# antoniorizzoeng/climate-sim-mpi-cpp

Measured on AMD Instinct MI355X. Metric: Mcell-updates/sec (16384^2 fp64 advection-diffusion sweep), higher is better.
Workload: dtype f64

## Files before the change

### climate-sim-mpi-cpp_amd/__init__.py

```python
from __future__ import annotations

import collections
import ctypes as C
import os
import subprocess
import weakref

import numpy as np

HERE = os.path.dirname(os.path.abspath(__file__))
ROOT = os.path.dirname(HERE)
LIB_PATH = os.environ.get("CSIM_LIB") or os.path.join(HERE, "lib", "libcsim.so")
HEADER = os.path.join(ROOT, "include", "csim.h")

DIRICHLET, NEUMANN, PERIODIC = 0, 1, 2
LEFT, RIGHT, BOTTOM, TOP = 0, 1, 2, 3
NO_NEIGHBOR = -1
UNIQUE_ID_BYTES = 128
VARIANTS = {"auto": 0, "dpp": 1, "lds": 2, "naive": 3}

_BC_NAMES = {
    "dirichlet": DIRICHLET, "fixed": DIRICHLET,
    "neumann": NEUMANN, "noflux": NEUMANN, "zero-flux": NEUMANN,
    "periodic": PERIODIC, "period": PERIODIC,
# ... 55 lines not shown

def lib() -> C.CDLL:
    global _lib
    if _lib is not None:
        return _lib
    if not os.path.exists(LIB_PATH):
        raise FileNotFoundError(
            f"{LIB_PATH} is missing: run __graft_entry__.build() (there is no CPU fallback)")
    if os.environ.get("CSIM_PRELOAD_TORCH", "1") != "0":
        try:
            import torch
        except Exception:
            pass
    L = C.CDLL(LIB_PATH, mode=C.RTLD_GLOBAL)
    dp, ip, vp = C.POINTER(C.c_double), C.POINTER(C.c_int), C.c_void_p
    d, i = C.c_double, C.c_int
    sig = {
        "csim_last_error": (C.c_char_p, []),
        "csim_abi_version": (i, []),
        "csim_device_count": (i, [ip]),
        "csim_set_device": (i, [i]),
        "csim_device_name": (i, [C.c_char_p, C.c_size_t]),
        "csim_safe_dt": (d, [d] * 5),
        "csim_decomp_init": (i, [i, i, i, i, C.POINTER(Decomp)]),
        "csim_exchange_plan": (i, [C.POINTER(Decomp), i, C.POINTER(Msg), ip, C.POINTER(Msg), ip]),
        "csim_field_create": (i, [i, i, i, d, d, C.POINTER(vp)]),
        "csim_field_destroy": (i, [vp]),
        "csim_field_upload": (i, [vp, dp]),
        "csim_field_download": (i, [vp, dp]),
        "csim_field_download_interior": (i, [vp, dp]),
        "csim_field_fill": (i, [vp, d]),
        "csim_field_copy": (i, [vp, vp]),
        "csim_field_swap": (i, [vp, vp]),
        "csim_field_minmax": (i, [vp, dp]),
        "csim_field_sum": (i, [vp, dp]),
        "csim_field_linf_diff": (i, [vp, vp, dp]),
        "csim_apply_boundary": (i, [vp, ip, ip, d]),
        "csim_diffusion_step": (i, [vp, vp, d, d]),
        "csim_advection_step": (i, [vp, vp, d, d, d]),
        "csim_fused_step": (i, [vp, vp, d, d, d, d]),
        "csim_stepper_create": (i, [C.POINTER(Decomp), d, d, ip, d, C.POINTER(vp)]),
        "csim_stepper_destroy": (i, [vp]),
        "csim_comm_unique_id": (i, [vp, C.c_size_t]),
        "csim_stepper_comm_init": (i, [vp, vp, C.c_size_t]),
        "csim_stepper_upload": (i, [vp, dp]),
        "csim_stepper_download": (i, [vp, dp]),
# ... 65 lines not shown
        "csim_obs_network_observe": (i, [vp, i, C.c_ulonglong, C.c_uint, i]),
        "csim_obs_noise": (i, [C.c_ulonglong, C.c_uint, C.c_uint, dp]),
        "csim_ensemble_assimilate_network": (i, [vp, vp, d, i, i]),
        "csim_obs_network_fetch": (i, [vp, dp, dp, dp, dp, dp, dp]),
        "csim_obs_network_log": (i, [vp, i, C.POINTER(CsimObsCycle), ip]),
        "csim_obs_network_log_reset": (i, [vp]),
        "csim_obs_network_create_linear": (i, [vp, i, ip, ip, ip, ip, ip, dp, dp, d, i, i, C.POINTER(vp)]),
        "csim_obs_network_taps": (i, [vp, ip]),
        "csim_obs_linear_check": (i, [i, i, i, i, i, ip, ip, ip, ip, ip, dp]),
        "csim_obs_taps_bilinear": (i, [i, i, d, d, ip, ip, ip, ip, dp]),
        "csim_obs_taps_box": (i, [i, i, i, i, i, i, ip, ip, ip, dp]),
        "csim_obs_network_set_active": (i, [vp, C.POINTER(C.c_ubyte)]),
        "csim_ensemble_assimilate_screened": (i, [vp, vp, d, i, i, d]),
        "csim_obs_network_screen_log": (i, [vp, i, C.POINTER(CsimObsScreenCycle), ip]),
        "csim_obs_network_status": (i, [vp, C.POINTER(C.c_ubyte)]),
        "csim_obs_screen_decide": (i, [d, d, d, d, d, i, ip]),
        "csim_ensemble_set_option": (i, [vp, C.c_char_p, C.c_long]),
        "csim_ensemble_get_option": (i, [vp, C.c_char_p, C.POINTER(C.c_long)]),
        "csim_ensemble_plan": (i, [i, i, i, i, ip]),
        "csim_ensemble_sign_class": (i, [d, d, d, d, d, d, i, ip]),
        "csim_ensemble_classes": (i, [i, ip, ip]),
    }
    for name, (res, args) in sig.items():
        fn = getattr(L, name)
        fn.restype = res
        fn.argtypes = args
    _lib = L
    return L


def declared_symbols():
    import re
    txt = open(HEADER).read()
    return sorted(set(re.findall(r"\b(csim_[a-z0-9_]+)\s*\(", txt)))


def _ck(rc):
    if rc != 0:
        raise CsimError(rc, lib().csim_last_error().decode())


def _dp(a):
    assert a.dtype == np.float64 and a.flags["C_CONTIGUOUS"]
    return a.ctypes.data_as(C.POINTER(C.c_double))


# ... 11 lines not shown
def bc_codes(code: str):
    m = {"d": DIRICHLET, "n": NEUMANN, "p": PERIODIC}
    return [m[c] for c in code.lower()]


def device_count() -> int:
    n = C.c_int(0)
    _ck(lib().csim_device_count(C.byref(n)))
    return n.value


def set_device(dev: int) -> None:
    _ck(lib().csim_set_device(dev))


def device_name() -> str:
    buf = C.create_string_buffer(256)
    _ck(lib().csim_device_name(buf, 256))
    return buf.value.decode()


def safe_dt(dx, dy, vx, vy, D) -> float:
    return lib().csim_safe_dt(dx, dy, vx, vy, D)


def decomp_init(size, rank, nx_global, ny_global) -> Decomp:
    d = Decomp()
    _ck(lib().csim_decomp_init(size, rank, nx_global, ny_global, C.byref(d)))
    return d


def exchange_plan(dec: Decomp, depth: int):
    sends, recvs = (Msg * 8)(), (Msg * 8)()
    ns, nr = C.c_int(0), C.c_int(0)
    _ck(lib().csim_exchange_plan(C.byref(dec), depth, sends, C.byref(ns), recvs, C.byref(nr)))
    return ([(m.peer, m.dir, m.count) for m in sends[:ns.value]],
            [(m.peer, m.dir, m.count) for m in recvs[:nr.value]])


def pass_schedule(nsteps: int, smallest_tile: int = 1 << 30, fuse: int = -1, tile_cells: int = 0, diffusion_only: bool = False):
    n = C.c_long(0)
    args = (nsteps, min(smallest_tile, 1 << 30), tile_cells, fuse, int(diffusion_only))
    _ck(lib().csim_pass_schedule_for(*args, None, 0, C.byref(n)))
    buf = (C.c_int * max(1, n.value))()
    _ck(lib().csim_pass_schedule_for(*args, buf, n.value, C.byref(n)))
    return list(buf[:n.value])
# ... 776 lines not shown
```

### climate-sim-mpi-cpp_amd/csrc/api.cpp

```cpp
#include "stepper.hpp"

namespace csim {

static thread_local std::string g_err;
int fail(int code, const std::string& msg) {
    g_err = msg;
    return code;
}
static bool pow2(double x) {
    if (!(x > 0.0) || !std::isnormal(x)) return false;
    int e = 0;
    return std::frexp(x, &e) == 0.5 && std::isnormal(1.0 / x);
}

Phys make_phys(double dx, double dy, double D, double dt, double vx, double vy, bool contract) {
    Phys p;
    p.kdiff = dt * D;
    p.mdt = -dt;
    p.vx = vx;
    p.vy = vy;
    p.dx = dx;
    p.dy = dy;
    p.dx2 = dx * dx;
    p.dy2 = dy * dy;
// ... 4 lines not shown
    if (dx == 1.0 && dy == 1.0)
        p.div_mode = 0;
    else if (pow2(dx) && pow2(dy) && pow2(p.dx2) && pow2(p.dy2))
        p.div_mode = 1;
    else
        p.div_mode = 2;
    {
        const long double kx = static_cast<long double>(dt) * D / (static_cast<long double>(dx) * dx);
        const long double ky = static_cast<long double>(dt) * D / (static_cast<long double>(dy) * dy);
        const long double cx = static_cast<long double>(dt) * vx / dx, cy = static_cast<long double>(dt) * vy / dy;
        const long double acx = cx < 0 ? -cx : cx, acy = cy < 0 ? -cy : cy;
        p.a0 = static_cast<double>(1.0L - 2.0L * kx - 2.0L * ky - acx - acy);
        p.aW = static_cast<double>(kx + (vx >= 0.0 ? acx : 0.0L));
        p.aE = static_cast<double>(kx + (vx >= 0.0 ? 0.0L : acx));
        p.aS = static_cast<double>(ky + (vy >= 0.0 ? acy : 0.0L));
        p.aN = static_cast<double>(ky + (vy >= 0.0 ? 0.0L : acy));
    }
    {
        const double g = (1.0 + 4.0 * std::fabs(p.kdiff) * (1.0 / p.dx2 + 1.0 / p.dy2) +
                          2.0 * std::fabs(p.mdt) * (std::fabs(vx) / std::fabs(dx) + std::fabs(vy) / std::fabs(dy))) * (1.0 + 1e-9);
        const double thr = std::ldexp(1.0, 1022) / std::pow(g, MAX_FUSE);
        p.fast_thr = (std::isfinite(g) && thr >= std::ldexp(1.0, 900)) ? thr : 0.0;
    }
    if (contract) p.div_mode = 3;
    return p;
}

int finish_partials(const double* scratch_dev, int nblocks, int kind, double out[2],
                           hipStream_t st) {
    std::vector<double> h(2 * REDUCE_BLOCKS);
    CSIM_HIP(hipMemcpyAsync(h.data(), scratch_dev, sizeof(double) * 2 * REDUCE_BLOCKS,
                            hipMemcpyDeviceToHost, st));
    CSIM_HIP(hipStreamSynchronize(st));
    double r0 = h[0], r1 = h[REDUCE_BLOCKS];
    for (int k = 1; k < nblocks; ++k) {
        if (kind == 0) {
            r0 = std::fmin(r0, h[k]);
            r1 = std::fmax(r1, h[REDUCE_BLOCKS + k]);
        } else if (kind == 1) {
            r0 += h[k];
        } else {
            r0 = max_nan(r0, h[k]);
        }
    }
    out[0] = r0;
    out[1] = r1;
// ... 51 lines not shown

const char* csim_last_error(void) { return g_err.c_str(); }

int csim_abi_version(void) { return CSIM_ABI_VERSION; }

int csim_device_count(int* count) {
    CSIM_REQUIRE(count, "count is null");
    CSIM_HIP(hipGetDeviceCount(count));
    return CSIM_OK;
}

int csim_set_device(int device) {
    CSIM_HIP(hipSetDevice(device));
    return CSIM_OK;
}

int csim_device_name(char* buf, size_t n) {
    CSIM_REQUIRE(buf && n > 0, "bad buffer");
    int dev = 0;
    CSIM_HIP(hipGetDevice(&dev));
    hipDeviceProp_t prop;
    CSIM_HIP(hipGetDeviceProperties(&prop, dev));
    std::snprintf(buf, n, "%s", prop.gcnArchName);
    return CSIM_OK;
}

double csim_safe_dt(double dx, double dy, double vx, double vy, double D) {
    const double inf = std::numeric_limits<double>::infinity();
    const double ax = std::fabs(vx), ay = std::fabs(vy);
    const double rate = (ax > 0 ? ax / dx : 0.0) + (ay > 0 ? ay / dy : 0.0);
    const double dt_adv = rate > 0 ? 1.0 / rate : inf;
    const double w = 1.0 / (dx * dx) + 1.0 / (dy * dy);
    const double dt_diff = D > 0 ? 1.0 / (2.0 * D * w) : inf;
    return std::min(dt_adv, dt_diff);
}

int csim_decomp_init(int size, int rank, int nx_global, int ny_global, csim_decomp* out) {
    CSIM_REQUIRE(out, "out is null");
    CSIM_REQUIRE(size >= 1 && rank >= 0 && rank < size, "bad size/rank");
    CSIM_REQUIRE(nx_global > 0 && ny_global > 0, "nx/ny must be > 0");
    int small = 1;
    for (int f = 1; static_cast<long>(f) * f <= size; ++f)
        if (size % f == 0) small = f;
    csim_decomp d{};
    d.size = size;
    d.rank = rank;
// ... 190 lines not shown
```

### climate-sim-mpi-cpp_amd/csrc/internal.hpp

```cpp
#pragma once

#include <hip/hip_runtime.h>

#include <cstddef>
#include <cstdio>
#include <string>

#include "csim.h"

namespace csim {

constexpr int LPAD = 16;
constexpr int WAVE_COLS = 128;

inline int round_up(int v, int m) { return (v + m - 1) / m * m; }
inline int pitch_for(int nx) { return LPAD + round_up(nx + 1, WAVE_COLS) + WAVE_COLS; }

int fail(int code, const std::string& msg);

#define CSIM_HIP(expr)                                                                       \
    do {                                                                                     \
        hipError_t e_ = (expr);                                                              \
        if (e_ != hipSuccess)                                                                \
            return ::csim::fail(CSIM_ERR_HIP, std::string(#expr) + ": " + hipGetErrorString(e_)); \
    } while (0)

struct Phys {
    double kdiff;
    double mdt;
    double vx, vy;
    double dx, dy;
    double dx2, dy2;
    double rdx, rdy, rdx2, rdy2;
    int div_mode;
    double a0, aW, aE, aS, aN;
    double fast_thr;
};
Phys make_phys(double dx, double dy, double D, double dt, double vx, double vy, bool contract = false);

enum { VAR_AUTO = 0, VAR_DPP = 1, VAR_LDS = 2, VAR_NAIVE = 3 };

struct SweepCfg {
    int variant = VAR_AUTO;
    int rows_per_chunk = 0;
    int tuned_rows = 0;
    int lds_bytes = 0;
    int prefetch = 0;
    int xcd_swizzle = 1;
    int tail_split = 1;
    int frame_rows = 0;
    int* rows_used = nullptr;
};

hipError_t launch_sweep(const double* in, double* out, int nx, int ny, int pitch, const Phys& p,
                        const SweepCfg& cfg, hipStream_t st);
struct FrameSync {
    unsigned* counter = nullptr;
    unsigned long long* flag = nullptr;
    unsigned long long pass = 0;
// ... 69 lines not shown
```

### climate-sim-mpi-cpp_amd/csrc/passes.cpp

```cpp
#include "stepper.hpp"

using namespace csim;

static int post_exchange2(csim_stepper* s, int H, hipStream_t st) { return post_plan(s, H, st); }
static hipError_t launch_fused(csim_stepper* s, const Phys& p, const int kind[4], int T, int part,
                               hipStream_t st, bool final_pass = false, int lds_bytes = 0,
                               const FrameSync* sync = nullptr) {
    SweepCfg cfg = s->cfg;
    if (lds_bytes > 0) cfg.lds_bytes = lds_bytes;
    if (T >= 2 && T <= MAX_FUSE && s->tuned_T[T] > 0) cfg.tuned_rows = s->tuned_T[T];
    cfg.rows_used = &s->last_rows;
    return launch_sweepO(s->cur, s->nxt, s->nx, s->ny, s->pitch, p, cfg, kind, s->bc_value, T, part, st,
                         final_pass ? s->fin : nullptr, sync);
}

static int pass_fused_bulk_first(csim_stepper* s, const Phys& p, int T, bool final_pass) {
    int kind[4];
    for (int k = 0; k < 4; ++k) kind[k] = s->phys[k] ? s->bc[k] : 3;
    GhostArgs g = ghost_args(s);
    for (int k = 0; k < 4; ++k) g.recv[k] = nullptr;
    s->pre_unpacked = false;
    hipStream_t X, Y;
    if (!s->relay || !s->s_relay[0]) {
        CSIM_SETTLE(s);
// ... 279 lines not shown
            best[idx] = std::min(best[idx], ms);
        }
    std::vector<size_t> order(cand.size());
    for (size_t c = 0; c < order.size(); ++c) order[c] = c;
    std::sort(order.begin(), order.end(), [&](size_t a, size_t b) { return best[a] < best[b]; });
    const size_t finalists = std::min<size_t>(4, order.size());
    for (int round = 0; round < 5; ++round)
        for (size_t q = 0; q < finalists; ++q) {
            const size_t idx = order[(round & 1) ? finalists - 1 - q : q];
            int rc = trial(cand[idx], &ms);
            if (rc) return rc;
            best[idx] = std::min(best[idx], ms);
        }
    size_t arg = order[0];
    for (size_t q = 1; q < finalists; ++q)
        if (best[order[q]] < best[arg]) arg = order[q];
    s->tuned_T[T] = cand[arg];
    if (preferred_depth) s->cfg.tuned_rows = cand[arg];
    return CSIM_OK;
}

}

static void note_flavour(csim_stepper* s, const Phys& p) {
    s->fused_2c_active = p.fast_thr > 0.0 && p.div_mode != 3;
    const int still = s->fused_2c_active && p.div_mode <= 1 && p.vx == 0.0 && p.vy == 0.0;
    if (still != s->diffusion_only_active) s->forget_tuning();
    s->diffusion_only_active = still;
}

extern "C" {

int csim_stepper_tune(csim_stepper* s, double D, double dt, double vx, double vy) {
    CSIM_REQUIRE(s, "null stepper");
    CSIM_SETTLE(s);
    Phys p = make_phys(s->dx, s->dy, D, dt, vx, vy, s->contract != 0);
    if (!s->fused_2c) p.fast_thr = 0.0;
    note_flavour(s, p);
    const int depth = fused_depth(s);
    if (depth < 2 || s->cfg.rows_per_chunk != 0) return CSIM_OK;
    if (!s->tuned) {
        int rc = tune_rows(s, p, depth);
        if (rc) return rc;
    }
    if (s->fuse < 0)
        for (int T = std::min(MAX_FUSE, s->fuse_cap); T >= 4; --T)
            if (T != depth && s->tuned_T[T] == 0) {
                int rc = tune_rows(s, p, T, false);
                if (rc) return rc;
            }
    return CSIM_OK;
}

int csim_stepper_keep_warm(csim_stepper* s, double D, double dt, double vx, double vy, double seconds) {
    CSIM_REQUIRE(s, "null stepper");
    CSIM_REQUIRE(seconds >= 0.0 && seconds <= 10.0, "seconds must be in [0, 10]");
    CSIM_SETTLE(s);
    const auto t0 = std::chrono::steady_clock::now();
    auto elapsed = [&] { return std::chrono::duration<double>(std::chrono::steady_clock::now() - t0).count(); };
    Phys p = make_phys(s->dx, s->dy, D, dt, vx, vy, s->contract != 0);
    if (!s->fused_2c) p.fast_thr = 0.0;
    note_flavour(s, p);
    const int depth = fused_depth(s);
    if (depth < 2) return CSIM_OK;
    int kind[4];
    for (int k = 0; k < 4; ++k) kind[k] = s->phys[k] ? s->bc[k] : 3;
    CSIM_HIP(hipStreamSynchronize(s->s_comm));
    CSIM_HIP(hipStreamSynchronize(s->s_comp));
    double last = 0.0;
    for (int n = 0; n < 100000; ++n) {
        const double before = elapsed();
        if (before + 1.25 * last >= seconds) break;
        CSIM_HIP(launch_sweepO(s->cur, s->nxt, s->nx, s->ny, s->pitch, p, s->cfg, kind, s->bc_value, depth, 0, s->s_comp));
        CSIM_HIP(hipStreamSynchronize(s->s_comp));
        last = elapsed() - before;
    }
    return CSIM_OK;
}

int csim_stepper_run(csim_stepper* s, double D, double dt, double vx, double vy, int nsteps) {
    CSIM_REQUIRE(s, "null stepper");
    CSIM_REQUIRE(nsteps >= 0, "nsteps must be >= 0");
    Phys p = make_phys(s->dx, s->dy, D, dt, vx, vy, s->contract != 0);
    if (!s->fused_2c) p.fast_thr = 0.0;
    note_flavour(s, p);
    const int depth = fused_depth(s);
    const bool can_fuse = depth >= 2;
    const bool auto_depth = s->fuse < 0;
    const int cap = !can_fuse ? 1 : auto_depth ? std::min(MAX_FUSE, s->fuse_cap) : depth;
    if (s->multi && s->external) {
        if (nsteps == 1 && !s->halo_fresh)
            return fail(CSIM_ERR_STATE, "external halo transport: csim_stepper_halo_unpack first");
        if (nsteps >= 2 && !(can_fuse && nsteps <= cap))
            return fail(CSIM_ERR_STATE, "external halo transport: a call advances 1 step or one fused pass");
    } else if (s->multi && !s->comm) {
        return fail(CSIM_ERR_STATE, "multi-rank stepper needs csim_stepper_comm_init before run");
    }
    if (!s->external && (s->faces_depth != 0 || s->pre_unpacked))
        return fail(CSIM_ERR_STATE, "internal: csim_stepper_run entered with faces of a fused pass in flight "
                                    "(an earlier call failed half-way?): upload or re-initialise the field");
    const GhostArgs g = ghost_args(s);
    if (s->multi && s->external && nsteps >= 2) return pass_fused(s, p, nsteps, 0);
    if (can_fuse && s->autotune && !s->tuned && s->cfg.rows_per_chunk == 0 && nsteps >= 4 * depth) {
        CSIM_SETTLE(s);
        int rc = tune_rows(s, p, depth);
        if (rc) return rc;
    }
// ... 26 lines not shown
```

### climate-sim-mpi-cpp_amd/csrc/stepper.cpp

```cpp
#include "stepper.hpp"

using namespace csim;

size_t csim_stepper::face_len(int d, int H) const { return face_doubles(d, H, nx, ny); }

namespace csim {

int settle(csim_stepper* s) {
    if (s->tail == nullptr || s->tail == s->s_comp) {
        s->tail = s->s_comp;
        return CSIM_OK;
    }
    CSIM_HIP(hipEventRecord(s->ev_tail, s->tail));
    CSIM_HIP(hipStreamWaitEvent(s->s_comp, s->ev_tail, 0));
    s->tail = s->s_comp;
    return CSIM_OK;
}

bool depth_ok(const csim_stepper* s, int depth) {
    return depth >= 2 && depth <= MAX_FUSE && depth <= s->nx && depth <= s->ny;
}

int fused_depth(const csim_stepper* s) {
    const int depth = std::min(s->fuse < 0 ? pref_fuse(s->tile_cells, s->diffusion_only_active != 0) : s->fuse, s->fuse_cap);
// ... 458 lines not shown
        if (!s->external && (s->faces_depth != 0 || s->pre_unpacked))
            return fail(CSIM_ERR_STATE, "internal: exchange schedule changed with faces of a fused pass in flight");
        if (value == 3 && s->multi && !s->frame_flag)
            return fail(CSIM_ERR_STATE, "overlap 3 needs hipStreamWaitValue64 / signal memory, which this device or runtime refused");
        s->overlap = static_cast<int>(value);
    } else if (k == "frame_fence") {
        CSIM_REQUIRE(value == 0 || value == 1, "frame_fence must be 0 or 1");
        s->frame_fence = static_cast<int>(value);
    } else if (k == "frame_rows") {
        CSIM_REQUIRE(value >= 0 && value <= 4096, "frame_rows must be 0..4096");
        s->cfg.frame_rows = static_cast<int>(value);
    } else if (k == "frame_prio") {
        s->frame_prio = value != 0;
    } else if (k == "relay") {
        CSIM_SETTLE(s);
        s->relay = value != 0;
    } else if (k == "relay_events") {
        CSIM_REQUIRE(value == 0 || value == 1, "relay_events must be 0 or 1");
        s->relay_events = static_cast<int>(value);
    } else if (k == "direct_faces") {
        s->direct_faces = value != 0;
    } else if (k == "fused_2c") {
        s->fused_2c = value != 0;
    } else if (k == "external_halo") {
        s->external = value != 0;
        s->halo_fresh = false;
    } else if (k == "contract") {
        CSIM_REQUIRE(value == 0 || value == 1, "contract must be 0 (reference operation order, default) or 1");
        if (s->contract != static_cast<int>(value)) s->forget_tuning();
        s->contract = static_cast<int>(value);
    } else if (k == "fuse") {
        CSIM_REQUIRE(value >= -1 && value <= MAX_FUSE, "fuse must be -1 (auto) or 0..7");
        s->fuse = static_cast<int>(value);
    } else if (k == "lds_bytes") {
        CSIM_REQUIRE(value >= 0 && value <= 65536, "lds_bytes must be 0..65536");
        s->cfg.lds_bytes = static_cast<int>(value);
    } else if (k == "autotune") {
        s->autotune = value != 0;
        s->forget_tuning();
    } else if (k == "tuned_rows" || k == "last_rows") {
        return fail(CSIM_ERR_ARG, k + " is read-only");
    } else if (k == "sync_timeout_ms") {
        CSIM_REQUIRE(value >= 0, "sync_timeout_ms must be >= 0");
        s->sync_timeout_ms = value;
    } else if (k == "test_stall") {
        CSIM_REQUIRE(value == 0 || value == 1, "test_stall must be 0 or 1");
// ... 16 lines not shown
        return fail(CSIM_ERR_ARG, "unknown option: " + k);
    }
    return CSIM_OK;
}

int csim_stepper_get_option(const csim_stepper* s, const char* key, long* value) {
    CSIM_REQUIRE(s && key && value, "null argument");
    const std::string k(key);
    if (k == "variant") *value = s->cfg.variant;
    else if (k == "rows_per_chunk") *value = s->cfg.rows_per_chunk;
    else if (k == "tuned_rows") *value = s->cfg.tuned_rows;
    else if (k.size() == 12 && k.compare(0, 11, "tuned_rows_") == 0 && k[11] >= '2' && k[11] <= '0' + MAX_FUSE)
        *value = s->tuned_T[k[11] - '0'];
    else if (k == "last_rows") *value = s->last_rows;
    else if (k == "prefetch") *value = s->cfg.prefetch;
    else if (k == "xcd_swizzle") *value = s->cfg.xcd_swizzle;
    else if (k == "tail_split") *value = s->cfg.tail_split;
    else if (k == "overlap") *value = s->overlap;
    else if (k == "direct_faces") *value = s->direct_faces;
    else if (k == "relay") *value = s->relay;
    else if (k == "relay_events") *value = s->relay_events;
    else if (k == "fused_2c") *value = s->fused_2c;
    else if (k == "fused_2c_active") *value = s->fused_2c_active;
    else if (k == "diffusion_only_active") *value = s->diffusion_only_active;
    else if (k == "frame_rows") *value = s->cfg.frame_rows;
    else if (k == "external_halo") *value = s->external;
    else if (k == "fuse") *value = s->fuse;
    else if (k == "contract") *value = s->contract;
    else if (k == "autotune") *value = s->autotune;
    else if (k == "profile") *value = s->profile;
    else if (k == "sync_timeout_ms") *value = s->sync_timeout_ms;
    else if (k == "test_stall") *value = s->stall_armed;
    else if (k == "faces_in_flight") *value = s->faces_depth != 0 || s->pre_unpacked;
    else return fail(CSIM_ERR_ARG, "unknown option: " + k);
    return CSIM_OK;
}

int csim_stepper_kernel_time(csim_stepper* s, int steps_per_launch, double* total_ms,
                             long* launches) {
    CSIM_REQUIRE(s && total_ms && launches, "null argument");
    CSIM_REQUIRE(steps_per_launch >= 1 && steps_per_launch <= MAX_FUSE, "steps_per_launch must be 1..7");
    int rc = prof_fold(s);
    if (rc) return rc;
    *total_ms = s->prof_ms[steps_per_launch];
    *launches = s->prof_launches[steps_per_launch];
    return CSIM_OK;
// ... 24 lines not shown
```

### climate-sim-mpi-cpp_amd/csrc/stepper.hpp

```cpp
#pragma once
#include <rccl/rccl.h>

#include <algorithm>
#include <chrono>
#include <cmath>
#include <cstring>
#include <limits>
#include <string>
#include <vector>

#include "internal.hpp"
#include "obs_taps.hpp"


#define CSIM_NCCL(expr)                                                                        \
    do {                                                                                       \
        ncclResult_t r_ = (expr);                                                              \
        if (r_ != ncclSuccess)                                                                 \
            return ::csim::fail(CSIM_ERR_RCCL, std::string(#expr) + ": " + ncclGetErrorString(r_)); \
    } while (0)

#define CSIM_REQUIRE(cond, msg) OBS_REQUIRE(cond, msg)


// ... 18 lines not shown
    hipEvent_t ev_relay_ready = nullptr, ev_relay_bulk = nullptr;
    int relay_events = 0;
    int relay = 1;
    hipEvent_t ev_edge = nullptr, ev_recv = nullptr, ev_ready = nullptr;
    ncclComm_t comm = nullptr;
    bool comm_borrowed = false;
    long sync_timeout_ms = 0;
    bool stall_armed = false;
    bool multi = false;
    bool halo_fresh = false;
    bool edge_async = false;
    int nbr8[8]{-1, -1, -1, -1, -1, -1, -1, -1};
    size_t cap2[8]{0, 0, 0, 0, 0, 0, 0, 0};
    size_t face_len(int d, int H) const;
    double* send2[8]{nullptr, nullptr, nullptr, nullptr, nullptr, nullptr, nullptr, nullptr};
    double* recv2[8]{nullptr, nullptr, nullptr, nullptr, nullptr, nullptr, nullptr, nullptr};
    hipEvent_t ev_edge2 = nullptr, ev_recv2 = nullptr;
    unsigned* frame_counter = nullptr;
    unsigned long long* frame_flag = nullptr;
    unsigned long long pass_no = 0;
    int frame_fence = 0, frame_prio = 1;
    int fused_2c = 1;
    int fused_2c_active = 0;
    int diffusion_only_active = 0;
    int direct_faces = 1;
    bool bulk_first_run = false;
    double* snap_d = nullptr;
    double* snap_h = nullptr;
    hipStream_t s_io = nullptr;
    hipEvent_t ev_snap_src = nullptr, ev_snap_copied = nullptr;
    bool snap_pending = false;
    int last_rows = 0;
    long tile_cells = 0;
    int fuse_cap = 1;
    int faces_depth = 0;
    csim::SweepCfg cfg;
    int overlap = 5;
    bool phys_ring_filled = false;
    bool ring_ok = false;
    bool pre_unpacked = false;
    int fuse = -1;
    int contract = 0;
    int external = 0;
    int profile = 0;
    bool prof_active = false;
    long prof_slot = -1;
// ... 70 lines not shown
```

### climate-sim-mpi-cpp_amd/csrc/sweepO.hpp

```cpp
#pragma once
#include "sweep_core.hpp"

#pragma clang fp contract(off)

namespace csim {

__device__ __forceinline__ void face_store_cell(const FrameSync& fs, int i, int j, double v, int nx, int ny) {
    const int H = fs.face_depth;
    const unsigned long long bits = static_cast<unsigned long long>(__double_as_longlong(v));
    auto put = [&](double* face, int idx) {
        __hip_atomic_store(reinterpret_cast<unsigned long long*>(face + idx), bits, __ATOMIC_RELAXED, __HIP_MEMORY_SCOPE_AGENT);
    };
    const bool in_i = i >= 1 && i <= nx, in_j = j >= 1 && j <= ny;
    const bool l = in_i && i <= H, r = in_i && i >= nx - H + 1, b = in_j && j <= H, t = in_j && j >= ny - H + 1;
    const int cl = i - 1, cr = i - (nx - H + 1), rb = j - 1, rt = j - (ny - H + 1);
    if (l && fs.face[0]) put(fs.face[0], cl * (ny + 2) + j);
    if (r && fs.face[1]) put(fs.face[1], cr * (ny + 2) + j);
    if (b && fs.face[2]) put(fs.face[2], rb * (nx + 2) + i);
    if (t && fs.face[3]) put(fs.face[3], rt * (nx + 2) + i);
    if (l && b && fs.face[4]) put(fs.face[4], rb * H + cl);
    if (r && b && fs.face[5]) put(fs.face[5], rb * H + cr);
    if (l && t && fs.face[6]) put(fs.face[6], rt * H + cl);
    if (r && t && fs.face[7]) put(fs.face[7], rt * H + cr);
}
// ... 67 lines not shown
        const bool rows = (kb != 3 && jb - (T - 1) < 1) || (kt != 3 && je + (T - 1) > ny);
        int col_case = 0;
        if (kl != 3 && kr != 3)
            col_case = 7;
        else if (kl != 3)
            col_case = kl == CSIM_BC_NEUMANN ? 2 : 1;
        else if (kr != 3)
            col_case = (kr == CSIM_BC_NEUMANN ? 5 : 3) + (nx & 1);
        if (!SPECIALISE_EDGES<DIV, T>::value || rows || col_case == 7) col_case = -1;
#define CSIM_MARCH(MODE_) \
    sweepO_march<DIV, T, MODE_, SX, SY>(in, out, nx, ny, pitch, jb, je, g0, lane, kl, kr, a.p, kb, kt, late, fin_frame, first, last, wt)
        switch (col_case) {
            case 0: if (SPECIALISE_EDGES<DIV, T>::value) CSIM_MARCH(0); break;
            case 1: if (SPECIALISE_EDGES<DIV, T>::value) CSIM_MARCH(1); break;
            case 2: if (SPECIALISE_EDGES<DIV, T>::value) CSIM_MARCH(2); break;
            case 3: if (SPECIALISE_EDGES<DIV, T>::value) CSIM_MARCH(3); break;
            case 4: if (SPECIALISE_EDGES<DIV, T>::value) CSIM_MARCH(4); break;
            case 5: if (SPECIALISE_EDGES<DIV, T>::value) CSIM_MARCH(5); break;
            case 6: if (SPECIALISE_EDGES<DIV, T>::value) CSIM_MARCH(6); break;
            default: CSIM_MARCH(M_GENERIC); break;
        }
    } else {
        bool redo = true;
        if (DIV != 3 && a.p.fast_thr > 0.0) redo = CSIM_MARCH(M_FAST);
        if (redo) {
            keep_branch();
            CSIM_MARCH(M_PLAIN);
        }
    }
#undef CSIM_MARCH
    if (signalling) {
        const LateArgs::Ptr ka = late.here();
        FrameSync fs;
        fs.counter = ka->fs.counter, fs.flag = ka->fs.flag, fs.pass = ka->fs.pass, fs.nframe = ka->fs.nframe;
        fs.fence = ka->fs.fence, fs.face_depth = ka->fs.face_depth;
#pragma unroll
        for (int d = 0; d < 8; ++d) fs.face[d] = ka->fs.face[d];
        if (fs.fence == 0)
            asm volatile("s_waitcnt vmcnt(0)" ::: "memory");
        if (fs.fence == 0 && fs.face_depth > 0) {
            const int H = fs.face_depth;
            const int gx = g0 + 2 * lane;
            const bool out_lane = 2 * lane >= TP && 2 * lane < TP + STRIDE && gx < nx;
            const bool rows_near = jb <= H || je >= ny - H + 1;
            const bool cols_near = g0 + TP < H || g0 + TP + STRIDE > nx - H;
            if (rows_near || cols_near) {
                const int jf0 = jb == 1 ? 0 : jb, jf1 = je == ny ? ny + 1 : je;
// ... 174 lines not shown
```

### climate-sim-mpi-cpp_amd/csrc/sweep_core.hpp

```cpp
#pragma once
#include <algorithm>
#include <type_traits>

#include "internal.hpp"

#pragma clang fp contract(off)

namespace csim {

template <int DIV, bool FAST = false>
__device__ __forceinline__ double diffuse_term(double c, double W, double E, double S, double N,
                                               const Phys& p) {
    double lx, ly;
    if (FAST) {
        lx = __builtin_fma(-2.0, c, E) + W;
        ly = __builtin_fma(-2.0, c, N) + S;
    } else {
        const double tc = 2.0 * c;
        lx = (E - tc) + W;
        ly = (N - tc) + S;
    }
    if (DIV == 1) {
        lx = lx * p.rdx2;
        ly = ly * p.rdy2;
// ... 12 lines not shown
    if (SX == 1)
        gx = c - W;
    else if (SX == 0)
        gx = E - c;
    else
        gx = (p.vx >= 0.0) ? (c - W) : (E - c);
    if (SY == 1)
        gy = c - S;
    else if (SY == 0)
        gy = N - c;
    else
        gy = (p.vy >= 0.0) ? (c - S) : (N - c);
    if (DIV == 1) {
        gx = gx * p.rdx;
        gy = gy * p.rdy;
    } else if (DIV == 2) {
        gx = gx / p.dx;
        gy = gy / p.dy;
    }
    const double adv = p.vx * gx + p.vy * gy;
    return p.mdt * adv;
}

template <int DIV, int SX = -1, int SY = -1, bool FAST = false>
__device__ __forceinline__ double cell(double c, double W, double E, double S, double N,
                                       const Phys& p) {
    if (DIV == 3) {
        double o = p.a0 * c;
        o = __builtin_fma(p.aW, W, o);
        o = __builtin_fma(p.aE, E, o);
        o = __builtin_fma(p.aS, S, o);
        return __builtin_fma(p.aN, N, o);
    }
    const double o = diffuse_term<DIV, FAST>(c, W, E, S, N, p);
    if (FAST && (SX == 2 || SY == 2)) {
        if (SX == 2 && SY == 2) return o;
        double g;
        if (SY == 2)
            g = SX == 1 ? c - W : E - c;
        else
            g = SY == 1 ? c - S : N - c;
        if (DIV == 1) g = g * (SY == 2 ? p.rdx : p.rdy);
        const double adv = (SY == 2 ? p.vx : p.vy) * g;
        return o + p.mdt * adv;
    }
    return o + advect_term<DIV, (SX == 2 ? 1 : SX), (SY == 2 ? 1 : SY)>(c, W, E, S, N, p);
}

__device__ __forceinline__ double from_prev_lane(double src, double edge) {
    int lo = __builtin_amdgcn_update_dpp(__double2loint(edge), __double2loint(src), 0x138, 0xf, 0xf, false);
    int hi = __builtin_amdgcn_update_dpp(__double2hiint(edge), __double2hiint(src), 0x138, 0xf, 0xf, false);
    return __hiloint2double(hi, lo);
}
__device__ __forceinline__ double from_next_lane(double src, double edge) {
    int lo = __builtin_amdgcn_update_dpp(__double2loint(edge), __double2loint(src), 0x130, 0xf, 0xf, false);
    int hi = __builtin_amdgcn_update_dpp(__double2hiint(edge), __double2hiint(src), 0x130, 0xf, 0xf, false);
    return __hiloint2double(hi, lo);
// ... 76 lines not shown
    __device__ __forceinline__ static LateArgs get() {
        typedef const char __attribute__((address_space(4))) * Bytes;
        LateArgs l;
        l.a = (Ptr)((Bytes)__builtin_amdgcn_kernarg_segment_ptr() + SWEEP_ARGS_KERNARG_OFFSET);
        return l;
    }
    __device__ __forceinline__ Ptr here() const {
        Ptr q = a;
        asm volatile("" : "+s"(q));
        return q;
    }
    __device__ __forceinline__ double* fin_line(int side) const { return here()->fin.line[side]; }
};

template <int T>
struct OverlapGeom {
    static constexpr int TP = 2 * ((T + 1) / 2);
    static constexpr int STRIDE = WAVE_COLS - 2 * TP;
};

__device__ __forceinline__ void pin(double& v) { asm volatile("" : "+v"(v)); }
__device__ __forceinline__ void pin2(double2& v) { asm volatile("" : "+v"(v.x), "+v"(v.y)); }

constexpr int M_FAST = -3, M_PLAIN = -2, M_GENERIC = -1;

template <int DIV, int T, int MODE, int SX, int SY>
__device__ __forceinline__ bool sweepO_march(const double* __restrict__ in, double* __restrict__ out,
                                             int nx, int ny, int pitch, int jb, int je, int g0, int lane,
                                             int kl, int kr, const Phys& p, int kb, int kt,
                                             LateArgs late, bool fin_any, bool fin_l, bool fin_r, bool wt) {
    constexpr int TP = OverlapGeom<T>::TP;
    constexpr int STRIDE = OverlapGeom<T>::STRIDE;
    constexpr bool EDGE = MODE >= M_GENERIC, FAST = MODE == M_FAST, GENERIC = MODE == M_GENERIC;
    constexpr int CASE = MODE;
    const int gx = g0 + 2 * lane, gy = gx + 1;
    const ptrdiff_t xoff = LPAD + gx;
    const bool out_lane = 2 * lane >= TP && 2 * lane < TP + STRIDE && gx < nx;
    const int nvalid = nx - gx;
    const bool ghost_ly = kl != 3 && gy == -1;
    const bool ghost_rx = kr != 3 && gx == nx, ghost_ry = kr != 3 && gy == nx;
    const bool right_in_x = (nx & 1) == 0;
    const bool ghost_cols = kl != 3 || kr != 3;

    auto load = [&](int j) {
        return *reinterpret_cast<const double2*>(in + static_cast<ptrdiff_t>(j) * pitch + xoff);
    };

    const int r_first = jb - (T - 1);
    const int niter = (je - jb + 1) + 2 * (T - 1);
    const int last_row = r_first + niter;
    double2 L0[6];
    double2 L[T][3];
#pragma unroll
    for (int q = 0; q < 6; ++q) L0[q] = load(min(r_first - 1 + q, last_row));
    bool big = false;
    auto screen = [&](const double2& v) {
        big |= !(__builtin_fabs(v.x) < p.fast_thr);
        big |= !(__builtin_fabs(v.y) < p.fast_thr);
        if (SX == 2 || SY == 2) {
            big |= __builtin_amdgcn_class(v.x, 0x20);
            big |= __builtin_amdgcn_class(v.y, 0x20);
        }
    };
    if (FAST) {
        screen(L0[0]);
        screen(L0[1]);
    }
#pragma unroll
    for (int l = 0; l < T; ++l)
#pragma unroll
        for (int q = 0; q < 3; ++q) L[l][q] = make_double2(0.0, 0.0);

    auto group = [&](auto gtag, int k0) {
        constexpr int G = decltype(gtag)::value;
        const bool rows_here = GENERIC && ((kb != 3 && k0 <= 2 * T - 2 - jb) || (kt != 3 && k0 + 5 >= ny + T - jb));
#pragma unroll
        for (int u = 0; u < 6; ++u) {
            {
                const int r = r_first + k0 + u;
#pragma unroll
                for (int l = 1; l <= T; ++l) {
                    if (G < 2 && 6 * G + u < 2 * (l - 1)) continue;
                    const int rho = r - l + 1;
                    const double2 s = (l == 1) ? L0[u % 6] : L[l - 1][(u + 1) % 3];
                    const double2 c = (l == 1) ? L0[(u + 1) % 6] : L[l - 1][(u + 2) % 3];
                    const double2 n = (l == 1) ? L0[(u + 2) % 6] : L[l - 1][u % 3];
                    double2 o;
                    {
                        const double Wx = shift_from_prev(c.y);
                        const double Ey = shift_from_next(c.x);
                        o.x = cell<DIV, SX, SY, FAST>(c.x, Wx, c.y, s.x, n.x, p);
                        o.y = cell<DIV, SX, SY, FAST>(c.y, c.x, Ey, s.y, n.y, p);
                        if (FAST && l == 1) screen(n);
                    }
                    if (EDGE && !GENERIC && l < T) {
                        if (CASE == 1) o.y = ghost_ly ? c.y : o.y;
                        if (CASE == 2) {
                            const double nb = shift_from_next(o.x);
                            o.y = ghost_ly ? nb : o.y;
                        }
                        if (CASE == 3) o.x = ghost_rx ? c.x : o.x;
                        if (CASE == 4) o.y = ghost_ry ? c.y : o.y;
                        if (CASE == 5) {
                            const double pb = shift_from_prev(o.y);
                            o.x = ghost_rx ? pb : o.x;
                        }
                        if (CASE == 6) o.y = ghost_ry ? o.x : o.y;
                    }
                    if (GENERIC && l < T) {
                        bool ghost_row = false;
                        if (rows_here) {
                            const bool gb = rho == 0 && kb != 3, gt = rho == ny + 1 && kt != 3;
                            ghost_row = gb || gt;
                            if (ghost_row) {
                                const int kk = gb ? kb : kt;
// ... 70 lines not shown
                        } else {
                            store_pair(out + static_cast<ptrdiff_t>(rho) * pitch + xoff, o.x, o.y, nvalid);
                        }
                    }
                }
                L0[u % 6] = load(min(r + 5, last_row));
            }
        }
    };
    using G2 = std::integral_constant<int, 2>;
    if (EDGE) {
        for (int k0 = 0; k0 < niter; k0 += 6) group(G2{}, k0);
    } else {
        group(std::integral_constant<int, 0>{}, 0);
        if (niter > 6) group(std::integral_constant<int, 1>{}, 6);
        for (int k0 = 12; k0 < niter; k0 += 6) group(G2{}, k0);
    }
    return FAST && __builtin_amdgcn_ballot_w64(big) != 0;
}

template <int DIV, int T>
struct SPECIALISE_EDGES {
    static constexpr bool value = (DIV == 0 || DIV == 1) && T >= 4;
};

struct GhostDev {
    int bc[4];
    int phys[4];
    double value;
    const double* recv[4];
    const double* adj[4];
    int ext_depth;
};

__device__ __forceinline__ size_t at(int i, int j, int pitch) {
    return static_cast<size_t>(j) * pitch + (LPAD - 1) + i;
}

__device__ __forceinline__ void ghost_fill_cell(double* __restrict__ a, double* __restrict__ b, int nx, int ny,
                                                int pitch, const GhostDev& g, int t) {
    auto put = [&](size_t o, double v) {
        a[o] = v;
        if (b) b[o] = v;
    };
    if (t < ny) {
        const int j = t + 1;
// ... 93 lines not shown
```

### include/csim.h

```cpp
#ifndef CSIM_H
#define CSIM_H

#include <stddef.h>

#ifdef __cplusplus
extern "C" {
#endif

#define CSIM_ABI_VERSION 1

enum {
    CSIM_OK = 0,
    CSIM_ERR_ARG = 1,
    CSIM_ERR_HIP = 2,
    CSIM_ERR_RCCL = 3,
    CSIM_ERR_STATE = 4,
    CSIM_ERR_UNSUPPORTED = 5,
    CSIM_ERR_TIMEOUT = 6
};

enum { CSIM_BC_DIRICHLET = 0, CSIM_BC_NEUMANN = 1, CSIM_BC_PERIODIC = 2 };
enum { CSIM_LEFT = 0, CSIM_RIGHT = 1, CSIM_BOTTOM = 2, CSIM_TOP = 3 };

#define CSIM_NO_NEIGHBOR (-1)
#define CSIM_UNIQUE_ID_BYTES 128

typedef struct csim_field csim_field;
typedef struct csim_stepper csim_stepper;

typedef struct csim_decomp {
    int size, rank;
    int dims[2];
    int coords[2];
    int nbr[4];
    int nx_global, ny_global;
    int nx_local, ny_local;
    int x_offset, y_offset;
} csim_decomp;

const char* csim_last_error(void);
int csim_abi_version(void);
int csim_device_count(int* count);
int csim_set_device(int device);
int csim_device_name(char* buf, size_t n);

double csim_safe_dt(double dx, double dy, double vx, double vy, double D);
int csim_decomp_init(int size, int rank, int nx_global, int ny_global, csim_decomp* out);
typedef struct csim_msg {
    int peer;
    int dir;
    long count;
} csim_msg;
int csim_exchange_plan(const csim_decomp* dec, int depth, csim_msg sends[8], int* nsend, csim_msg recvs[8],
                       int* nrecv);

int csim_field_create(int nx, int ny, int halo, double dx, double dy, csim_field** out);
int csim_field_destroy(csim_field* f);
int csim_field_upload(csim_field* f, const double* host_with_ghosts);
int csim_field_download(const csim_field* f, double* host_with_ghosts);
int csim_field_download_interior(const csim_field* f, double* host_ny_by_nx);
int csim_field_fill(csim_field* f, double value);
int csim_field_copy(csim_field* dst, const csim_field* src);
int csim_field_swap(csim_field* a, csim_field* b);
int csim_field_minmax(const csim_field* f, double out_min_max[2]);
int csim_field_sum(const csim_field* f, double* out);
int csim_field_linf_diff(const csim_field* a, const csim_field* b, double* out);

int csim_apply_boundary(csim_field* f, const int bc[4], const int is_physical[4], double value);
int csim_diffusion_step(const csim_field* u, csim_field* out, double D, double dt);
// ... 149 lines not shown
```

Before: 1.594 million.

## Add power-of-two velocity fast path with exact single-FMA upwind advection

When both velocity components (scaled by the grid spacing) are exact powers of two, the upwind advection term is rewritten as one FMA with a precomputed ratio q and a single multiply by K. Because scaling by a power of two is exact, this matches the original rounding as long as values stay inside a screened range. The screen now also flags small nonzero values below a subnormal-safety threshold, and flagged tiles fall back to the plain path. It is on by default only for grids of at least 60M cells. The cost is extra per-value screen comparisons and a further kernel specialisation.

```diff
diff --git a/climate-sim-mpi-cpp_amd/__init__.py b/climate-sim-mpi-cpp_amd/__init__.py
--- a/climate-sim-mpi-cpp_amd/__init__.py
+++ b/climate-sim-mpi-cpp_amd/__init__.py
@@ -101,6 +101,7 @@
         "csim_set_device": (i, [i]),
         "csim_device_name": (i, [C.c_char_p, C.c_size_t]),
         "csim_safe_dt": (d, [d] * 5),
+        "csim_pow2_velocity_screen": (i, [d] * 6 + [C.POINTER(d)]),
         "csim_decomp_init": (i, [i, i, i, i, C.POINTER(Decomp)]),
         "csim_exchange_plan": (i, [C.POINTER(Decomp), i, C.POINTER(Msg), ip, C.POINTER(Msg), ip]),
         "csim_field_create": (i, [i, i, i, d, d, C.POINTER(vp)]),
@@ -212,6 +213,8 @@
         "csim_ensemble_classes": (i, [i, ip, ip]),
     }
     for name, (res, args) in sig.items():
+        if name == "csim_pow2_velocity_screen" and os.environ.get("CSIM_LIB") and not hasattr(L, name):
+            continue
         fn = getattr(L, name)
         fn.restype = res
         fn.argtypes = args
@@ -269,6 +272,12 @@
 
 def safe_dt(dx, dy, vx, vy, D) -> float:
     return lib().csim_safe_dt(dx, dy, vx, vy, D)
+
+
+def pow2_velocity_screen(D, dt, vx, vy, dx=1.0, dy=1.0):
+    out = (C.c_double * 4)()
+    _ck(lib().csim_pow2_velocity_screen(dx, dy, D, dt, vx, vy, out))
+    return tuple(out)
 
 
 def decomp_init(size, rank, nx_global, ny_global) -> Decomp:
diff --git a/climate-sim-mpi-cpp_amd/csrc/api.cpp b/climate-sim-mpi-cpp_amd/csrc/api.cpp
--- a/climate-sim-mpi-cpp_amd/csrc/api.cpp
+++ b/climate-sim-mpi-cpp_amd/csrc/api.cpp
@@ -50,6 +50,32 @@
         const double thr = std::ldexp(1.0, 1022) / std::pow(g, MAX_FUSE);
         p.fast_thr = (std::isfinite(g) && thr >= std::ldexp(1.0, 900)) ? thr : 0.0;
     }
+    p.slow_thr = p.p2_hi = p.p2_q = p.p2_k = 0.0;
+    if (!contract && p.div_mode <= 1 && p.fast_thr > 0.0 && pow2(std::fabs(vx)) && pow2(std::fabs(vy)) && std::isfinite(p.kdiff) &&
+        std::isfinite(p.mdt)) {
+        const double A = p.div_mode == 1 ? vx * p.rdx : vx, B = p.div_mode == 1 ? vy * p.rdy : vy;
+        if (pow2(std::fabs(A)) && pow2(std::fabs(B))) {
+            const bool by_y = vy > 0.0 || vx < 0.0;
+            const double q = by_y ? A / B : B / A, K = p.mdt * (by_y ? B : A);
+            const int eA = std::ilogb(A), eB = std::ilogb(B), eq = std::ilogb(q);
+            int e2 = 0, ew = std::min({0, eA, eB, eq, -eq}), eh = std::max({0, eA, eB, eq, -eq});
+            if (p.div_mode == 1) {
+                e2 = std::min({0, std::ilogb(p.rdx2), std::ilogb(p.rdy2)});
+                ew = std::min({ew, e2, std::ilogb(p.rdx), std::ilogb(p.rdy)});
+                eh = std::max({eh, std::ilogb(p.rdx), std::ilogb(p.rdy)});
+            }
+            int er = 0;
+            if (p.kdiff != 0.0) er = std::min(er, std::ilogb(p.kdiff) - 52 + e2);
+            if (p.mdt != 0.0) er = std::min(er, std::ilogb(p.mdt) - 52 + std::min(eA, eB));
+            const int eL = -1074 + 52 - MAX_FUSE * er - ew;
+            if (eL <= -300 && eh <= 100 && pow2(std::fabs(q)) && (K == 0.0 || std::isnormal(K))) {
+                p.slow_thr = std::ldexp(1.0, eL);
+                p.p2_hi = std::ldexp(p.fast_thr, -(eh + 2));
+                p.p2_q = q;
+                p.p2_k = K;
+            }
+        }
+    }
     if (contract) p.div_mode = 3;
     return p;
 }
@@ -147,6 +173,13 @@
     hipDeviceProp_t prop;
     CSIM_HIP(hipGetDeviceProperties(&prop, dev));
     std::snprintf(buf, n, "%s", prop.gcnArchName);
+    return CSIM_OK;
+}
+
+int csim_pow2_velocity_screen(double dx, double dy, double D, double dt, double vx, double vy, double out[4]) {
+    CSIM_REQUIRE(out, "null argument");
+    const Phys p = make_phys(dx, dy, D, dt, vx, vy);
+    out[0] = p.slow_thr, out[1] = p.p2_hi, out[2] = p.p2_q, out[3] = p.p2_k;
     return CSIM_OK;
 }
 
diff --git a/climate-sim-mpi-cpp_amd/csrc/internal.hpp b/climate-sim-mpi-cpp_amd/csrc/internal.hpp
--- a/climate-sim-mpi-cpp_amd/csrc/internal.hpp
+++ b/climate-sim-mpi-cpp_amd/csrc/internal.hpp
@@ -35,6 +35,9 @@
     int div_mode;
     double a0, aW, aE, aS, aN;
     double fast_thr;
+    double slow_thr;
+    double p2_hi;
+    double p2_q, p2_k;
 };
 Phys make_phys(double dx, double dy, double D, double dt, double vx, double vy, bool contract = false);
 
diff --git a/climate-sim-mpi-cpp_amd/csrc/passes.cpp b/climate-sim-mpi-cpp_amd/csrc/passes.cpp
--- a/climate-sim-mpi-cpp_amd/csrc/passes.cpp
+++ b/climate-sim-mpi-cpp_amd/csrc/passes.cpp
@@ -325,8 +325,14 @@
 
 }
 
+constexpr long P2_MIN_CELLS = 60000000L;
+static bool pow2_v_wanted(const csim_stepper* s) {
+    return s->pow2_v == 1 || (s->pow2_v == 2 && static_cast<long>(s->nx) * s->ny >= P2_MIN_CELLS);
+}
+
 static void note_flavour(csim_stepper* s, const Phys& p) {
     s->fused_2c_active = p.fast_thr > 0.0 && p.div_mode != 3;
+    s->pow2_v_active = s->fused_2c_active && p.slow_thr > 0.0;
     const int still = s->fused_2c_active && p.div_mode <= 1 && p.vx == 0.0 && p.vy == 0.0;
     if (still != s->diffusion_only_active) s->forget_tuning();
     s->diffusion_only_active = still;
@@ -339,6 +345,7 @@
     CSIM_SETTLE(s);
     Phys p = make_phys(s->dx, s->dy, D, dt, vx, vy, s->contract != 0);
     if (!s->fused_2c) p.fast_thr = 0.0;
+    if (!s->fused_2c || !pow2_v_wanted(s)) p.slow_thr = 0.0;
     note_flavour(s, p);
     const int depth = fused_depth(s);
     if (depth < 2 || s->cfg.rows_per_chunk != 0) return CSIM_OK;
@@ -363,6 +370,7 @@
     auto elapsed = [&] { return std::chrono::duration<double>(std::chrono::steady_clock::now() - t0).count(); };
     Phys p = make_phys(s->dx, s->dy, D, dt, vx, vy, s->contract != 0);
     if (!s->fused_2c) p.fast_thr = 0.0;
+    if (!s->fused_2c || !pow2_v_wanted(s)) p.slow_thr = 0.0;
     note_flavour(s, p);
     const int depth = fused_depth(s);
     if (depth < 2) return CSIM_OK;
@@ -386,6 +394,7 @@
     CSIM_REQUIRE(nsteps >= 0, "nsteps must be >= 0");
     Phys p = make_phys(s->dx, s->dy, D, dt, vx, vy, s->contract != 0);
     if (!s->fused_2c) p.fast_thr = 0.0;
+    if (!s->fused_2c || !pow2_v_wanted(s)) p.slow_thr = 0.0;
     note_flavour(s, p);
     const int depth = fused_depth(s);
     const bool can_fuse = depth >= 2;
diff --git a/climate-sim-mpi-cpp_amd/csrc/stepper.cpp b/climate-sim-mpi-cpp_amd/csrc/stepper.cpp
--- a/climate-sim-mpi-cpp_amd/csrc/stepper.cpp
+++ b/climate-sim-mpi-cpp_amd/csrc/stepper.cpp
@@ -504,6 +504,11 @@
         s->direct_faces = value != 0;
     } else if (k == "fused_2c") {
         s->fused_2c = value != 0;
+    } else if (k == "pow2_v") {
+        CSIM_REQUIRE(value >= 0 && value <= 2, "pow2_v must be 0 (off), 1 (on) or 2 (on where it pays: large tiles)");
+        s->pow2_v = static_cast<int>(value);
+    } else if (k == "pow2_v_active") {
+        return fail(CSIM_ERR_ARG, k + " is read-only");
     } else if (k == "external_halo") {
         s->external = value != 0;
         s->halo_fresh = false;
@@ -566,6 +571,8 @@
     else if (k == "relay_events") *value = s->relay_events;
     else if (k == "fused_2c") *value = s->fused_2c;
     else if (k == "fused_2c_active") *value = s->fused_2c_active;
+    else if (k == "pow2_v") *value = s->pow2_v;
+    else if (k == "pow2_v_active") *value = s->pow2_v_active;
     else if (k == "diffusion_only_active") *value = s->diffusion_only_active;
     else if (k == "frame_rows") *value = s->cfg.frame_rows;
     else if (k == "external_halo") *value = s->external;
diff --git a/climate-sim-mpi-cpp_amd/csrc/stepper.hpp b/climate-sim-mpi-cpp_amd/csrc/stepper.hpp
--- a/climate-sim-mpi-cpp_amd/csrc/stepper.hpp
+++ b/climate-sim-mpi-cpp_amd/csrc/stepper.hpp
@@ -64,6 +64,8 @@
     int frame_fence = 0, frame_prio = 1;
     int fused_2c = 1;
     int fused_2c_active = 0;
+    int pow2_v = 2;
+    int pow2_v_active = 0;
     int diffusion_only_active = 0;
     int direct_faces = 1;
     bool bulk_first_run = false;
diff --git a/climate-sim-mpi-cpp_amd/csrc/sweepO.hpp b/climate-sim-mpi-cpp_amd/csrc/sweepO.hpp
--- a/climate-sim-mpi-cpp_amd/csrc/sweepO.hpp
+++ b/climate-sim-mpi-cpp_amd/csrc/sweepO.hpp
@@ -113,7 +113,18 @@
         }
     } else {
         bool redo = true;
-        if (DIV != 3 && a.p.fast_thr > 0.0) redo = CSIM_MARCH(M_FAST);
+        if (DIV != 3 && a.p.fast_thr > 0.0) {
+            if constexpr (P2_BODY<DIV, T, SX, SY>::value) {
+                if (a.p.slow_thr > 0.0) {
+                    keep_branch();
+                    redo = CSIM_MARCH(M_FAST_P2);
+                } else {
+                    redo = CSIM_MARCH(M_FAST);
+                }
+            } else {
+                redo = CSIM_MARCH(M_FAST);
+            }
+        }
         if (redo) {
             keep_branch();
             CSIM_MARCH(M_PLAIN);
diff --git a/climate-sim-mpi-cpp_amd/csrc/sweep_core.hpp b/climate-sim-mpi-cpp_amd/csrc/sweep_core.hpp
--- a/climate-sim-mpi-cpp_amd/csrc/sweep_core.hpp
+++ b/climate-sim-mpi-cpp_amd/csrc/sweep_core.hpp
@@ -58,7 +58,7 @@
     return p.mdt * adv;
 }
 
-template <int DIV, int SX = -1, int SY = -1, bool FAST = false>
+template <int DIV, int SX = -1, int SY = -1, bool FAST = false, bool P2 = false>
 __device__ __forceinline__ double cell(double c, double W, double E, double S, double N,
                                        const Phys& p) {
     if (DIV == 3) {
@@ -69,6 +69,13 @@
         return __builtin_fma(p.aN, N, o);
     }
     const double o = diffuse_term<DIV, FAST>(c, W, E, S, N, p);
+    if (P2) {
+        static_assert(!P2 || (FAST && DIV <= 1 && (SX == 0 || SX == 1) && (SY == 0 || SY == 1)), "see P2 above");
+        const double gx = SX == 1 ? c - W : E - c;
+        const double gy = SY == 1 ? c - S : N - c;
+        const double F = (SY == 1 || SX == 0) ? __builtin_fma(p.p2_q, gx, gy) : __builtin_fma(p.p2_q, gy, gx);
+        return o + p.p2_k * F;
+    }
     if (FAST && (SX == 2 || SY == 2)) {
         if (SX == 2 && SY == 2) return o;
         double g;
@@ -191,7 +198,7 @@
 __device__ __forceinline__ void pin(double& v) { asm volatile("" : "+v"(v)); }
 __device__ __forceinline__ void pin2(double2& v) { asm volatile("" : "+v"(v.x), "+v"(v.y)); }
 
-constexpr int M_FAST = -3, M_PLAIN = -2, M_GENERIC = -1;
+constexpr int M_FAST_P2 = -4, M_FAST = -3, M_PLAIN = -2, M_GENERIC = -1;
 
 template <int DIV, int T, int MODE, int SX, int SY>
 __device__ __forceinline__ bool sweepO_march(const double* __restrict__ in, double* __restrict__ out,
@@ -200,7 +207,7 @@
                                              LateArgs late, bool fin_any, bool fin_l, bool fin_r, bool wt) {
     constexpr int TP = OverlapGeom<T>::TP;
     constexpr int STRIDE = OverlapGeom<T>::STRIDE;
-    constexpr bool EDGE = MODE >= M_GENERIC, FAST = MODE == M_FAST, GENERIC = MODE == M_GENERIC;
+    constexpr bool EDGE = MODE >= M_GENERIC, P2 = MODE == M_FAST_P2, FAST = MODE == M_FAST || P2, GENERIC = MODE == M_GENERIC;
     constexpr int CASE = MODE;
     const int gx = g0 + 2 * lane, gy = gx + 1;
     const ptrdiff_t xoff = LPAD + gx;
@@ -224,9 +231,13 @@
     for (int q = 0; q < 6; ++q) L0[q] = load(min(r_first - 1 + q, last_row));
     bool big = false;
     auto screen = [&](const double2& v) {
-        big |= !(__builtin_fabs(v.x) < p.fast_thr);
-        big |= !(__builtin_fabs(v.y) < p.fast_thr);
-        if (SX == 2 || SY == 2) {
+        big |= !(__builtin_fabs(v.x) < (P2 ? p.p2_hi : p.fast_thr));
+        big |= !(__builtin_fabs(v.y) < (P2 ? p.p2_hi : p.fast_thr));
+        if (P2) {
+            big |= __builtin_fabs(v.x) < p.slow_thr && v.x != 0.0;
+            big |= __builtin_fabs(v.y) < p.slow_thr && v.y != 0.0;
+        }
+        if (SX == 2 || SY == 2 || (P2 && SX == 0 && SY == 0)) {
             big |= __builtin_amdgcn_class(v.x, 0x20);
             big |= __builtin_amdgcn_class(v.y, 0x20);
         }
@@ -258,8 +269,8 @@
                     {
                         const double Wx = shift_from_prev(c.y);
                         const double Ey = shift_from_next(c.x);
-                        o.x = cell<DIV, SX, SY, FAST>(c.x, Wx, c.y, s.x, n.x, p);
-                        o.y = cell<DIV, SX, SY, FAST>(c.y, c.x, Ey, s.y, n.y, p);
+                        o.x = cell<DIV, SX, SY, FAST, P2>(c.x, Wx, c.y, s.x, n.x, p);
+                        o.y = cell<DIV, SX, SY, FAST, P2>(c.y, c.x, Ey, s.y, n.y, p);
                         if (FAST && l == 1) screen(n);
                     }
                     if (EDGE && !GENERIC && l < T) {
@@ -376,6 +387,11 @@
 template <int DIV, int T>
 struct SPECIALISE_EDGES {
     static constexpr bool value = (DIV == 0 || DIV == 1) && T >= 4;
+};
+
+template <int DIV, int T, int SX, int SY>
+struct P2_BODY {
+    static constexpr bool value = SPECIALISE_EDGES<DIV, T>::value && (SX == 0 || SX == 1) && (SY == 0 || SY == 1);
 };
 
 struct GhostDev {
diff --git a/include/csim.h b/include/csim.h
--- a/include/csim.h
+++ b/include/csim.h
@@ -45,6 +45,7 @@
 int csim_device_name(char* buf, size_t n);
 
 double csim_safe_dt(double dx, double dy, double vx, double vy, double D);
+int csim_pow2_velocity_screen(double dx, double dy, double D, double dt, double vx, double vy, double out[4]);
 int csim_decomp_init(int size, int rank, int nx_global, int ny_global, csim_decomp* out);
 typedef struct csim_msg {
     int peer;
```

Result: faster. 1.715 million, median of 6 (+7.6%).
